# akhilsathuluri/sim_a_splat

Hardware: AMD Instinct MI355X
Metric: rendered frames/sec at 1M Gaussians 1920x1080 (higher is better)
Workload: dtype f32

## Files before the change

### sim_a_splat_amd/csrc/sas_api.cpp

```cpp
#include "../../include/sim_a_splat_amd.h"
#include "sas_internal.h"

#include <cmath>
#include <cstdarg>
#include <cstdio>
#include <cstdlib>
#include <cstring>
#include <algorithm>
#include <new>
#include <string>
#include <vector>

#pragma clang fp contract(off)

namespace {

template <class T, auto Free>
struct Owned {
    T h{};
    Owned() = default;
    Owned(Owned &&o) noexcept : h(o.h) { o.h = T{}; }
    Owned &operator=(Owned &&o) noexcept { std::swap(h, o.h); return *this; }
    ~Owned() { if (h) (void)Free(h); }
    T *put() { return &h; }
    operator T() const { return h; }
};
using Stream = Owned<hipStream_t, hipStreamDestroy>;
using Event = Owned<hipEvent_t, hipEventDestroy>;
template <class T> using Pinned = Owned<T *, hipHostFree>;

struct DevBuf {
    void *p = nullptr;
    size_t bytes = 0;
    DevBuf() = default;
    DevBuf(DevBuf &&o) noexcept : p(o.p), bytes(o.bytes) { o.p = nullptr; o.bytes = 0; }
    DevBuf &operator=(DevBuf &&o) noexcept { std::swap(p, o.p); std::swap(bytes, o.bytes); return *this; }
    ~DevBuf() { (void)release(); }
    int release(sas_ctx *c = nullptr);
};

struct ViewOut {
    float *rgb = nullptr, *alpha = nullptr, *depth = nullptr;
    uint8_t *rgb8 = nullptr;
    float *points = nullptr;
    uint8_t *mask = nullptr;
    uint8_t *rgb8_host = nullptr;
    float *features = nullptr;
    uint8_t *labels = nullptr;
    const uint8_t *lift_labels = nullptr;
    int64_t *lift_votes = nullptr, *lift_seen = nullptr;
    int lift_n = 0;
};

struct RenderArgs {
    float viewmat[16], K[9], bg[3];
// ... 213 lines not shown

uint32_t hilbert3(uint32_t x, uint32_t y, uint32_t z, int bits)
{
    uint32_t X[3] = {x, y, z};
    const uint32_t M = 1u << (bits - 1);
    for (uint32_t Q = M; Q > 1; Q >>= 1) {
        const uint32_t P = Q - 1;
        for (int i = 0; i < 3; ++i) {
            if (X[i] & Q) X[0] ^= P;
            else { const uint32_t t = (X[0] ^ X[i]) & P; X[0] ^= t; X[i] ^= t; }
        }
    }
    X[1] ^= X[0];
    X[2] ^= X[1];
    uint32_t t = 0;
    for (uint32_t Q = M; Q > 1; Q >>= 1)
        if (X[2] & Q) t ^= Q - 1;
    for (int i = 0; i < 3; ++i) X[i] ^= t;
    uint32_t code = 0;
    for (int b = bits - 1; b >= 0; --b)
        for (int i = 0; i < 3; ++i) code = (code << 1) | ((X[i] >> b) & 1u);
    return code;
}

void storage_order(int64_t n, const float *means, const uint8_t *gid, std::vector<int> &perm)
{
    perm.resize((size_t)n);
    float lo[3] = {INFINITY, INFINITY, INFINITY}, hi[3] = {-INFINITY, -INFINITY, -INFINITY};
    for (int64_t i = 0; i < n; ++i)
        for (int k = 0; k < 3; ++k) {
            const float v = means[3 * i + k];
            if (std::isfinite(v)) { lo[k] = std::min(lo[k], v); hi[k] = std::max(hi[k], v); }
        }
    float inv[3];
    for (int k = 0; k < 3; ++k) inv[k] = (hi[k] > lo[k]) ? 1023.0f / (hi[k] - lo[k]) : 0.0f;
    std::vector<uint64_t> key((size_t)n);
    for (int64_t i = 0; i < n; ++i) {
        uint32_t q[3];
        for (int k = 0; k < 3; ++k) {
            const float v = means[3 * i + k];
            float u = std::isfinite(v) ? (v - lo[k]) * inv[k] : 0.0f;
            u = std::min(std::max(u, 0.0f), 1023.0f);
            q[k] = (uint32_t)u;
        }
        const uint64_t g = gid ? gid[i] : 0;
        key[(size_t)i] = (g << 32) | hilbert3(q[0], q[1], q[2], 10);
    }
    for (int64_t i = 0; i < n; ++i) perm[(size_t)i] = (int)i;
    std::sort(perm.begin(), perm.end(), [&](int a, int b) { return key[a] != key[b] ? key[a] < key[b] : a < b; });
}

void make_cam(const float *V, const float *K, int W, int H, int tile_px, SasCam &c)
{
    for (int i = 0; i < 3; ++i) {
        for (int j = 0; j < 3; ++j) c.R[3 * i + j] = V[4 * i + j];
        c.t[i] = V[4 * i + 3];
    }
    for (int i = 0; i < 3; ++i) {
        float d = fmaf(c.R[6 + i], c.t[2], fmaf(c.R[3 + i], c.t[1], c.R[0 + i] * c.t[0]));
        c.campos[i] = -d;
    }
    c.fx = K[0]; c.fy = K[4]; c.cx = K[2]; c.cy = K[5];
    c.W = W; c.H = H;
    c.tile_px = tile_px;
    c.tw = (W + tile_px - 1) / tile_px;
    c.th = (H + tile_px - 1) / tile_px;
    c.Wf = (float)W; c.Hf = (float)H;
    const float tan_fovx = (0.5f * c.Wf) / c.fx;
    const float tan_fovy = (0.5f * c.Hf) / c.fy;
    c.lim_x_pos = fmaf(0.3f, tan_fovx, (c.Wf - c.cx) / c.fx);
    c.lim_x_neg = fmaf(0.3f, tan_fovx, c.cx / c.fx);
    c.lim_y_pos = fmaf(0.3f, tan_fovy, (c.Hf - c.cy) / c.fy);
    c.lim_y_neg = fmaf(0.3f, tan_fovy, c.cy / c.fy);
}

static size_t f_wg_stride(const sas_ctx *c) { return (((size_t)((c->scene.n + 255) / 256) + 3) & ~(size_t)3) + 4; }

int tiles_of(const Slot &sl) { return sl.cam.tw * sl.cam.th; }

long long frame_cap(const Slot &sl) { return sl.direct ? (long long)tiles_of(sl) * sl.scr.seg : sl.scr.cap; }

size_t key_slots(const Slot &sl) { return (size_t)std::max(frame_cap(sl), sl.scr.cap); }

long long grown(long long need, long long slack) { return need + need / 4 + slack; }

SasFrame frame_of(sas_ctx *c, Slot &sl, bool keep_info = false)
{
    Scratch &q = sl.scr;
    const int tiles = tiles_of(sl);
    SasFrame f{};
    f.rec = (float4 *)q.rec.p;
    f.col = (float4 *)q.col.p;
    f.info = (uint4 *)q.info.p;
    f.tickets = (unsigned *)q.counters.p;
    f.stats = (unsigned *)q.counters.p + SAS_TICKET_INTS;
    f.class_cursor = (int *)q.counters.p + SAS_TICKET_INTS + 8;
    f.stats_host = sl.stats_host;
    f.tile_count = (int *)q.counters.p + SAS_TICKET_INTS + 32;
    f.tile_big = f.tile_count + sas_count_stride(tiles);
    f.wg_base = (int *)q.wgbase.p;
    const size_t ts = sas_tile_stride(tiles);
    f.tile_offset = (int *)q.tilebuf.p;
    f.tile_cursor = (int *)q.tilebuf.p + ts;
    f.tile_order = (int *)q.tilebuf.p + 2 * ts;
    f.sort_class = (int *)q.tilebuf.p + 3 * ts;
    f.keys = (unsigned long long *)q.keys.p;
// ... 560 lines not shown
    if (n > 0 && (!means || !opacities || !colors)) return fail(c, SAS_ERR_INVALID, "means/opacities/colors required");
    const bool quat_mode = quats && scales;
    if (n > 0 && !quat_mode && !cov6) return fail(c, SAS_ERR_INVALID, "need quats+scales or cov6");
    if (n_groups < 0 || n_groups > 256) return fail(c, SAS_ERR_INVALID, "n_groups %d out of [0,256]", n_groups);
    if (group_id && n_groups <= 0) return fail(c, SAS_ERR_INVALID, "group_id given but n_groups == 0");
    HIP_TRY(c, hipSetDevice(c->device));
    if (const int rc = complete_all(c)) return rc;
    forget(c, HAVE_SCENE);

    const int deg = sh_degree < 0 ? -1 : sh_degree;
    const int coeff_floats = deg < 0 ? 3 : 3 * (deg + 1) * (deg + 1);
    const int planes = (coeff_floats + 3) / 4;
    const int64_t n_pad = (n + 63) & ~63ll;
    int rc;
    const size_t np = (size_t)(n_pad > 0 ? n_pad : 64);
    if ((rc = ensure(c, c->g0, sizeof(float4) * np))) return rc;
    if ((rc = ensure(c, c->g1, sizeof(float4) * np))) return rc;
    if ((rc = ensure(c, c->g2, sizeof(float4) * np))) return rc;
    if ((rc = ensure(c, c->col, sizeof(float4) * np * planes))) return rc;
    if ((rc = ensure(c, c->gid8, np))) return rc;

    c->perm_host.clear();
    if ((rc = ensure(c, c->perm, sizeof(int) * np))) return rc;
    if (n > 0) {
        std::vector<float> h_means((size_t)3 * n);
        std::vector<uint8_t> h_gid;
        HIP_TRY(c, hipMemcpy(h_means.data(), means, sizeof(float) * 3 * n, hipMemcpyDefault));
        if (group_id) {
            h_gid.resize((size_t)n);
            HIP_TRY(c, hipMemcpy(h_gid.data(), group_id, (size_t)n, hipMemcpyDefault));
            for (int64_t i = 0; i < n; ++i)
                if (h_gid[(size_t)i] >= n_groups) return fail(c, SAS_ERR_INVALID, "group_id[%lld]=%d >= n_groups=%d", (long long)i, (int)h_gid[(size_t)i], n_groups);
        }
        storage_order(n, h_means.data(), group_id ? h_gid.data() : nullptr, c->perm_host);
        HIP_TRY(c, hipMemcpy(c->perm.p, c->perm_host.data(), sizeof(int) * n, hipMemcpyHostToDevice));

        DevBuf s_means, s_q, s_s, s_cov, s_op, s_col, s_gid;
        auto stage = [&](DevBuf &b, const void *src, size_t bytes) -> int {
            if (const int rc = ensure(c, b, bytes)) return rc;
            HIP_TRY(c, hipMemcpy(b.p, src, bytes, hipMemcpyDefault));
            return SAS_OK;
        };
        rc = stage(s_means, means, sizeof(float) * 3 * n);
        if (!rc && quat_mode) rc = stage(s_q, quats, sizeof(float) * 4 * n);
        if (!rc && quat_mode) rc = stage(s_s, scales, sizeof(float) * 3 * n);
        if (!rc && !quat_mode) rc = stage(s_cov, cov6, sizeof(float) * 6 * n);
        if (!rc) rc = stage(s_op, opacities, sizeof(float) * n);
        if (!rc) rc = stage(s_col, colors, sizeof(float) * (size_t)coeff_floats * n);
        if (!rc && group_id) rc = stage(s_gid, group_id, (size_t)n);
        if (!rc) {
            sas_launch_relayout(nullptr, n, n_pad, (const int *)c->perm.p, (const float *)s_means.p,
                                (const float *)s_q.p, (const float *)s_s.p, (const float *)s_cov.p,
                                (const float *)s_op.p, (const float *)s_col.p, coeff_floats, planes,
                                (const uint8_t *)s_gid.p, (float4 *)c->g0.p, (float4 *)c->g1.p, (float4 *)c->g2.p,
                                (float4 *)c->col.p, (uint8_t *)c->gid8.p);
            hipError_t e = hipDeviceSynchronize();
            if (e != hipSuccess) rc = fail(c, SAS_ERR_HIP, "relayout: %s", hipGetErrorString(e));
        }
        if (rc) return rc;
    }

    c->scene = SasScene{};
    c->scene.g0 = (const float4 *)c->g0.p;
    c->scene.g1 = (const float4 *)c->g1.p;
    c->scene.g2 = (const float4 *)c->g2.p;
    c->scene.col = (const float4 *)c->col.p;
    c->scene.gid8 = (const uint8_t *)c->gid8.p;
    c->scene.perm = (const int *)c->perm.p;
    c->scene.n = n;
    c->scene.n_pad = n_pad;
    c->scene.sh_degree = deg;
    c->scene.cov_mode = quat_mode ? 0 : 1;
    c->scene.n_groups = group_id ? n_groups : 0;
    c->group_host.clear();
    c->links = LinkConsts{};
    if (group_id) {
        c->group_host.assign((size_t)12 * n_groups, 0.0f);
        for (int g = 0; g < n_groups; ++g) c->group_host[12 * g + 0] = c->group_host[12 * g + 5] = c->group_host[12 * g + 10] = 1.0f;
    }
    for (Slot &sl : c->slots) sl.scr.cap = 0;
    c->has_frame = false;
    c->scene_version++;
    c->have |= HAVE_SCENE;
    return SAS_OK;
}

int sas_set_group_poses(sas_ctx *c, int n_groups, const float *Rt)
{
    if (!c || !Rt) return SAS_ERR_INVALID;
    if (!has(c, HAVE_SCENE)) return fail(c, SAS_ERR_NO_SCENE, "no scene uploaded");
    if (n_groups != c->scene.n_groups) return fail(c, SAS_ERR_INVALID, "scene has %d groups, got %d", c->scene.n_groups, n_groups);
    c->group_host.assign(Rt, Rt + (size_t)12 * n_groups);
    return SAS_OK;
}

namespace {

void quat_to_matrix(const double *qin, double *R)
{
    const double n = std::sqrt(qin[0] * qin[0] + qin[1] * qin[1] + qin[2] * qin[2] + qin[3] * qin[3]);
    const double q[4] = {qin[0] / n, qin[1] / n, qin[2] / n, qin[3] / n};
    double qq[4][4];
    for (int a = 0; a < 4; ++a)
        for (int b = 0; b < 4; ++b) qq[a][b] = q[a] * q[b];
    R[0] = 1 - 2 * (qq[2][2] + qq[3][3]); R[1] = 2 * (qq[1][2] - qq[0][3]); R[2] = 2 * (qq[1][3] + qq[0][2]);
    R[3] = 2 * (qq[1][2] + qq[0][3]); R[4] = 1 - 2 * (qq[1][1] + qq[3][3]); R[5] = 2 * (qq[2][3] - qq[0][1]);
    R[6] = 2 * (qq[1][3] - qq[0][2]); R[7] = 2 * (qq[2][3] + qq[0][1]); R[8] = 1 - 2 * (qq[1][1] + qq[2][2]);
}

void matrix_to_quat(const double *R, double *q)
{
    const double tr = R[0] + R[4] + R[8];
    if (tr > 0) {
        const double s = std::sqrt(tr + 1.0) * 2;
        q[0] = 0.25 * s; q[1] = (R[7] - R[5]) / s; q[2] = (R[2] - R[6]) / s; q[3] = (R[3] - R[1]) / s;
    } else {
        int i = 0;
        if (R[4] > R[0]) i = 1;
        if (R[8] > R[4 * i]) i = 2;
        const int j = (i + 1) % 3, k = (i + 2) % 3;
        const double s = std::sqrt(1.0 + R[4 * i] - R[4 * j] - R[4 * k]) * 2;
        q[0] = (R[3 * k + j] - R[3 * j + k]) / s;
        q[1 + i] = 0.25 * s;
        q[1 + j] = (R[3 * j + i] + R[3 * i + j]) / s;
        q[1 + k] = (R[3 * k + i] + R[3 * i + k]) / s;
// ... 1126 lines not shown
```

### sim_a_splat_amd/csrc/sas_device.h

```cpp
#pragma once
#include "sas_internal.h"

#pragma clang fp contract(off)

#define DEV __device__ __forceinline__

constexpr float kNear = 0.01f, kFar = 1e10f, kEps2d = 0.3f;
constexpr float kAlphaThr = 1.0f / 255.0f, kMaxAlpha = 0.999f, kTStop = 1e-4f;

DEV float fma_(float a, float b, float c) { return __builtin_fmaf(a, b, c); }
DEV float finite_colour(float v) { return fminf(fmaxf(v, -3.402823466e38f), 3.402823466e38f); }
DEV unsigned mbcnt64(unsigned long long m) { return __builtin_amdgcn_mbcnt_hi((unsigned)(m >> 32), __builtin_amdgcn_mbcnt_lo((unsigned)m, 0u)); }

#ifdef SAS_DEBUG_BOUNDS
static __device__ unsigned long long g_sas_bounds[4];
DEV bool sas_in_bounds(long long i, long long n, int code)
{
    if (i >= 0 && i < n) return true;
    if (atomicAdd(&g_sas_bounds[0], 1ull) == 0ull) {
        g_sas_bounds[1] = (unsigned long long)code;
        g_sas_bounds[2] = (unsigned long long)i;
        g_sas_bounds[3] = (unsigned long long)n;
    }
    return false;
// ... 65 lines not shown
    unsigned u = __float_as_uint(x);
    int e = (int)(u >> 23) - 127;
    float m = __uint_as_float((u & 0x007fffffu) | 0x3f800000u);
    if (m > 1.41421356237f) { m = m * 0.5f; e += 1; }
    float s = (m - 1.0f) / (m + 1.0f);
    float s2 = s * s;
    float p = 0.1111111111f;
    p = fma_(p, s2, 0.1428571429f);
    p = fma_(p, s2, 0.2f);
    p = fma_(p, s2, 0.3333333333f);
    p = fma_(p, s2, 1.0f);
    float lnm = (2.0f * s) * p;
    return fma_((float)e, 0.6931471805599453f, lnm);
}

DEV float affine3(float r0, float r1, float r2, float t, float v0, float v1, float v2)
{
    return fma_(r0, v0, fma_(r1, v1, fma_(r2, v2, t)));
}
DEV float dot3(float a0, float a1, float a2, float b0, float b1, float b2)
{
    return fma_(a2, b2, fma_(a1, b1, a0 * b0));
}
DEV void pose_point(const float *G, float *p)
{
    const float x = affine3(G[0], G[1], G[2], G[3], p[0], p[1], p[2]);
    const float y = affine3(G[4], G[5], G[6], G[7], p[0], p[1], p[2]);
    const float z = affine3(G[8], G[9], G[10], G[11], p[0], p[1], p[2]);
    p[0] = x; p[1] = y; p[2] = z;
}
DEV void to_camera(const SasCam &c, const float *p, float *q)
{
    q[0] = affine3(c.R[0], c.R[1], c.R[2], c.t[0], p[0], p[1], p[2]);
    q[1] = affine3(c.R[3], c.R[4], c.R[5], c.t[1], p[0], p[1], p[2]);
    q[2] = affine3(c.R[6], c.R[7], c.R[8], c.t[2], p[0], p[1], p[2]);
}

DEV void rot_sym3(const float *R, const float *s, float *out)
{
    const float S[3][3] = {{s[0], s[1], s[2]}, {s[1], s[3], s[4]}, {s[2], s[4], s[5]}};
    float T[3][3];
#pragma unroll
    for (int i = 0; i < 3; ++i)
#pragma unroll
        for (int j = 0; j < 3; ++j)
            T[i][j] = dot3(R[3 * i + 0], R[3 * i + 1], R[3 * i + 2], S[0][j], S[1][j], S[2][j]);
    out[0] = dot3(T[0][0], T[0][1], T[0][2], R[0], R[1], R[2]);
    out[1] = dot3(T[0][0], T[0][1], T[0][2], R[3], R[4], R[5]);
    out[2] = dot3(T[0][0], T[0][1], T[0][2], R[6], R[7], R[8]);
    out[3] = dot3(T[1][0], T[1][1], T[1][2], R[3], R[4], R[5]);
    out[4] = dot3(T[1][0], T[1][1], T[1][2], R[6], R[7], R[8]);
    out[5] = dot3(T[2][0], T[2][1], T[2][2], R[6], R[7], R[8]);
}
```

### sim_a_splat_amd/csrc/sas_internal.h

```cpp
#pragma once
#include <hip/hip_runtime.h>
#include <stdint.h>

#define SAS_TILE 16
#define SAS_RS 2
#define SAS_CS 1
#define SAS_MAX_GROUP 4

struct SasCam {
    float R[9], t[3];
    float campos[3];
    float fx, fy, cx, cy;
    float lim_x_pos, lim_x_neg, lim_y_pos, lim_y_neg;
    float Wf, Hf;
    int W, H, tw, th;
    int tile_px;
};

struct SasScene {
    const float4 *g0, *g1, *g2, *col;
    const uint8_t *gid8;
    const int *perm;
    int64_t n;
    int64_t n_pad;
    int sh_degree;
    int cov_mode;
    int n_groups;
};

struct SasFrame {
    float4 *rec;
    float4 *col;
    uint4 *info;
    int *tile_count;
    int *tile_big;
    int *wg_base;
    int *class_cursor;
    int *tile_offset;
    int *tile_cursor;
    int *tile_order;
    int *sort_class;
    unsigned long long *keys;
    int *sorted_ids;
    long long cap;
    int seg;
    int cull;
    int group_fill;
    int keep_info;
    unsigned *stats;
    unsigned *tickets;
    unsigned *stats_host;
    int *wg_vis;
    int *wg_isect16;
    unsigned *tile_max;
    const float *group_Rt;
    const float *group_host;
    int n_wg;
    int n_tiles;
};

struct SasOutputs {
    float *rgb, *alpha, *depth;
    uint8_t *rgb8;
    uint8_t *rgb8_host;
    float bg[3];
    float *points;
    uint8_t *mask;
    float max_depth;
    int use_max_depth;
    long long n_pixels;
};
// ... 28 lines not shown
};
void sas_launch_pose_upload(hipStream_t st, const SasPoseUpload &u);

struct SasHostCopy {
    int nv;
    const uint8_t *src[SAS_MAX_GROUP];
    uint8_t *dst[SAS_MAX_GROUP];
    size_t bytes;
};
void sas_launch_host_copy(hipStream_t st, const SasHostCopy &h);

#define SAS_FEAT_K 8
#define SAS_MAX_FEATURES 256
struct SasFeatures {
    const float *store;
    float *out;
    long long n_pad;
    int C, chunks;
    float bg[SAS_MAX_FEATURES];
};
static inline int sas_feature_chunks(int C) { return (C + SAS_FEAT_K - 1) / SAS_FEAT_K; }
void sas_launch_feature_store(hipStream_t st, int64_t n, int64_t n_pad, const int *perm, const uint8_t *gid8, const float *src,
                              int C, float *store);
struct SasMeshFeatures {
    const unsigned long long *win;
    const float *store;
    long long nt;
};
void sas_launch_blend_features(hipStream_t st, const SasScene &s, int tiles, const SasParams &P, const SasFrame &f,
                               const SasFeatures &F, bool fast_exp, const SasMeshFeatures *MF);
struct SasLabels {
    const float *store;
    long long n_pad;
    int C, chunks;
    uint8_t *out;
    float min_alpha;
    int surface;
};
void sas_launch_blend_labels(hipStream_t st, const SasScene &s, int tiles, const SasParams &P, const SasFrame &f, const SasLabels &B,
                             bool fast_exp, const SasMeshFeatures *MF);
struct SasLift {
    const uint8_t *labels;
    unsigned long long *votes;
    unsigned long long *seen;
    long long n;
    int n_labels;
};
void sas_launch_lift_labels(hipStream_t st, const SasScene &s, int tiles, const SasParams &P, const SasFrame &f, const SasLift &B,
                            bool fast_exp);
void sas_launch_mesh_feature_store(hipStream_t st, int64_t nt, const int4 *tri, const float *src, int C, float *store);

void sas_launch_relayout(hipStream_t st, int64_t n, int64_t n_pad, const int *perm, const float *means, const float *quats,
                         const float *scales, const float *cov6, const float *opac, const float *colors,
                         int coeff_floats, int planes, const uint8_t *gid, float4 *g0, float4 *g1, float4 *g2,
                         float4 *col, uint8_t *gid8);
void sas_launch_project(hipStream_t st, const SasScene &s, const SasParams &P, const SasFrame &f);
void sas_launch_project2(hipStream_t st, const SasScene &s, const SasParams &P0, const SasFrame &f0, const SasParams &P1,
                         const SasFrame &f1);
void sas_launch_project_multi(hipStream_t st, const SasScene &s, const SasMulti &mf);
void sas_launch_scatter_multi(hipStream_t st, const SasScene &s, int tw, const SasMulti &mf);
void sas_launch_tiles_lazy_multi(hipStream_t st, const SasScene &s, int tiles, const SasMulti &mf, bool fast_exp, bool want_max,
                                 bool quad, hipEvent_t ev_start, hipEvent_t ev_stop);
void sas_launch_scatter(hipStream_t st, const SasScene &s, int tw, const SasFrame &f);
struct SasSortStreams {
    hipStream_t side[2];
    hipEvent_t fork, join[2];
};
void sas_launch_sort(hipStream_t st, const SasScene &s, int tiles, const SasFrame &f, const SasSortStreams &ss);
void sas_launch_blend(hipStream_t st, const SasScene &s, int tiles, const SasParams &P, const SasFrame &f,
                      bool fast_exp, bool want_max);
bool sas_tiles_lazy_quad_ok(bool fast_exp);
void sas_launch_tiles_lazy(hipStream_t st, const SasScene &s, int tiles, const SasParams &P, const SasFrame &f,
                           bool fast_exp, bool want_max, bool quad, hipEvent_t ev_start, hipEvent_t ev_stop);
void sas_launch_depth_tail(hipStream_t st, int tiles, const SasParams &P, const SasFrame &f, bool fill, bool points);
#define SAS_TICKET_INTS (65 * 32)
#define SAS_WIN_BINS 2048
static inline size_t sas_count_stride(int tiles) { return (((size_t)tiles + 1 + 1023) & ~(size_t)1023) + 1024; }
static inline size_t sas_counter_ints(int tiles) { return SAS_TICKET_INTS + 32 + 2 * sas_count_stride(tiles); }
static inline size_t sas_tile_stride(int tiles) { return ((size_t)tiles + 1 + 3) & ~(size_t)3; }

struct SasMeshScene {
    const float4 *vert;
    const int4 *tri;
    const float4 *color;
    int nv, nt;
    int n_groups;
    float ka, kd;
    const float4 *vnormal;
    const float4 *vcolor;
};
struct SasMeshFrame {
    float4 *rec;
    int4 *rect;
    int *tile_count;
    int *tile_offset;
    int *tile_cursor;
    int *list;
    long long cap;
    int n_rec;
    unsigned *status_host;
};
struct SasMeshExtra {
    unsigned long long *win;
    int surface;
};
#define SAS_MESH_PLANE_STRIDE 3
void sas_launch_mesh_bin(hipStream_t st, const SasMeshScene &m, const SasParams &P, const SasFrame &f, const SasMeshFrame &mf,
// ... 102 lines not shown
```

### sim_a_splat_amd/csrc/sas_kernels.hip

```cpp
#include "sas_device.h"

#include <cstdlib>
#include <cstring>
#include <type_traits>

#pragma clang fp contract(off)

namespace {

__global__ __launch_bounds__(256) void k_relayout(int64_t n, int64_t n_pad, const int *perm, const float *means,
                                                  const float *quats, const float *scales, const float *cov6,
                                                  const float *opac, const float *colors, int coeff_floats, int planes,
                                                  const uint8_t *gid, float4 *g0, float4 *g1, float4 *g2, float4 *col, uint8_t *gid8)
{
    const int64_t j = (int64_t)blockIdx.x * 256 + threadIdx.x;
    if (j >= n) return;
    const int64_t i = perm[j];
    float gbits = __uint_as_float(gid ? (unsigned)gid[i] : 0u);
    gid8[j] = gid ? gid[i] : (uint8_t)0;
    g0[j] = make_float4(means[3 * i], means[3 * i + 1], means[3 * i + 2], opac[i]);
    if (quats) {
        g1[j] = make_float4(quats[4 * i], quats[4 * i + 1], quats[4 * i + 2], quats[4 * i + 3]);
        g2[j] = make_float4(scales[3 * i], scales[3 * i + 1], scales[3 * i + 2], gbits);
    } else {
        const float *c = cov6 + 6 * i;
        g1[j] = make_float4(c[0], c[1], c[2], c[3]);
        g2[j] = make_float4(c[4], c[5], 0.0f, gbits);
    }
    const float *src = colors + (int64_t)coeff_floats * i;
    for (int p = 0; p < planes; ++p) {
        float v[4];
#pragma unroll
        for (int k = 0; k < 4; ++k) v[k] = (4 * p + k < coeff_floats) ? src[4 * p + k] : 0.0f;
        col[(int64_t)p * n_pad + j] = make_float4(v[0], v[1], v[2], v[3]);
    }
}

template <int DEG>
DEV void sh_to_color(const float *sh, float dx, float dy, float dz, float *rgb)
{
    float inorm = 1.0f / sqrtf(fma_(dz, dz, fma_(dy, dy, dx * dx)));
    float x = dx * inorm, y = dy * inorm, z = dz * inorm;
    float r[3];
#pragma unroll
    for (int c = 0; c < 3; ++c) r[c] = 0.2820947917738781f * sh[0 * 3 + c];
    if constexpr (DEG >= 1) {
#pragma unroll
        for (int c = 0; c < 3; ++c) {
            float t = fma_(-x, sh[3 * 3 + c], fma_(z, sh[2 * 3 + c], (-y) * sh[1 * 3 + c]));
            r[c] = fma_(0.48860251190292f, t, r[c]);
        }
    }
    float z2 = z * z;
    float fC1 = fma_(x, x, -(y * y));
    float fS1 = 2.0f * x * y;
    if constexpr (DEG >= 2) {
        float fTmp0B = -1.092548430592079f * z;
        float pSH6 = fma_(0.9461746957575601f, z2, -0.3153915652525201f);
        float pSH7 = fTmp0B * x;
        float pSH5 = fTmp0B * y;
        float pSH8 = 0.5462742152960395f * fC1;
        float pSH4 = 0.5462742152960395f * fS1;
#pragma unroll
        for (int c = 0; c < 3; ++c) {
            r[c] = fma_(pSH4, sh[4 * 3 + c], r[c]);
            r[c] = fma_(pSH5, sh[5 * 3 + c], r[c]);
            r[c] = fma_(pSH6, sh[6 * 3 + c], r[c]);
            r[c] = fma_(pSH7, sh[7 * 3 + c], r[c]);
            r[c] = fma_(pSH8, sh[8 * 3 + c], r[c]);
        }
    }
    if constexpr (DEG >= 3) {
        float fTmp0C = fma_(-2.285228997322329f, z2, 0.4570457994644658f);
        float fTmp1B = 1.445305721320277f * z;
        float fC2 = fma_(x, fC1, -(y * fS1));
        float fS2 = fma_(x, fS1, y * fC1);
        float pSH12 = z * fma_(1.865881662950577f, z2, -1.119528997770346f);
        float pSH13 = fTmp0C * x;
        float pSH11 = fTmp0C * y;
        float pSH14 = fTmp1B * fC1;
        float pSH10 = fTmp1B * fS1;
// ... 131 lines not shown
};

DEV Window window_of(int X0, int Y0, int X1, int Y1)
{
    Window w;
    w.X0 = X0; w.Y0 = Y0;
    w.ww = X1 - X0;
    w.area = (X1 > X0 && Y1 > Y0) ? w.ww * (Y1 - Y0) : 0;
    w.fits = w.area > 0 && w.area <= kHistBins;
    return w;
}

DEV Window wg_window(bool part, int x0, int x1, int y0, int y1, int *s_win)
{
    int mnx = part ? x0 : 0x7fffffff, mny = part ? y0 : 0x7fffffff;
    int mxx = part ? x1 : 0, mxy = part ? y1 : 0;
    mnx = wave_min_i32(mnx); mny = wave_min_i32(mny);
    mxx = wave_max_i32(mxx); mxy = wave_max_i32(mxy);
    if (threadIdx.x == 0) { s_win[0] = 0x7fffffff; s_win[1] = 0x7fffffff; s_win[2] = 0; s_win[3] = 0; }
    __syncthreads();
    if ((threadIdx.x & 63) == 0) {
        atomicMin(&s_win[0], mnx); atomicMin(&s_win[1], mny);
        atomicMax(&s_win[2], mxx); atomicMax(&s_win[3], mxy);
    }
    __syncthreads();
    return window_of(s_win[0], s_win[1], s_win[2], s_win[3]);
}

DEV Window wg_window_zeroed(bool part, int x0, int x1, int y0, int y1, int *s_win16, int *s_hist)
{
    int mnx = part ? x0 : 0x7fffffff, mny = part ? y0 : 0x7fffffff;
    int mxx = part ? x1 : 0, mxy = part ? y1 : 0;
    mnx = wave_min_i32(mnx); mny = wave_min_i32(mny);
    mxx = wave_max_i32(mxx); mxy = wave_max_i32(mxy);
    if ((threadIdx.x & 63) == 0) *reinterpret_cast<int4 *>(s_win16 + 4 * (threadIdx.x >> 6)) = make_int4(mnx, mny, mxx, mxy);
    static_assert(kHistBins == 2048, "eight bins per thread");
    reinterpret_cast<int4 *>(s_hist)[threadIdx.x] = make_int4(0, 0, 0, 0);
    reinterpret_cast<int4 *>(s_hist)[256 + threadIdx.x] = make_int4(0, 0, 0, 0);
    __syncthreads();
    const int4 a = reinterpret_cast<const int4 *>(s_win16)[0], b = reinterpret_cast<const int4 *>(s_win16)[1],
               c = reinterpret_cast<const int4 *>(s_win16)[2], d = reinterpret_cast<const int4 *>(s_win16)[3];
    return window_of(min(min(a.x, b.x), min(c.x, d.x)), min(min(a.y, b.y), min(c.y, d.y)),
                     max(max(a.z, b.z), max(c.z, d.z)), max(max(a.w, b.w), max(c.w, d.w)));
}

DEV bool mean_survives(float cz, float op) { return !(cz < kNear || cz > kFar) && !(op < kAlphaThr); }

struct ViewGeom {
    bool vis;
    int x0, x1, y0, y1;
    float mx, my, ca, cb, ccn, thr, z, rx, ry;
};

DEV void project_view(const SasCam &c, const float *cov, float op, float x, float y, float z, ViewGeom &g)
{
    float cc3[6];
    rot_sym3(c.R, cov, cc3);

    const float rz = 1.0f / z;
    const float rz2 = rz * rz;
    const float tx = z * fminf(c.lim_x_pos, fmaxf(-c.lim_x_neg, x * rz));
    const float ty = z * fminf(c.lim_y_pos, fmaxf(-c.lim_y_neg, y * rz));
    const float ja = c.fx * rz, jb = -((c.fx * tx) * rz2);
    const float jc = c.fy * rz, jd = -((c.fy * ty) * rz2);
    const float t00 = fma_(jb, cc3[2], ja * cc3[0]);
    const float t01 = fma_(jb, cc3[4], ja * cc3[1]);
    const float t02 = fma_(jb, cc3[5], ja * cc3[2]);
    const float t11 = fma_(jd, cc3[4], jc * cc3[3]);
    const float t12 = fma_(jd, cc3[5], jc * cc3[4]);
    float c00 = fma_(t02, jb, t00 * ja);
    const float c01 = fma_(t02, jd, t01 * jc);
    float c11 = fma_(t12, jd, t11 * jc);
    const float mx = fma_(c.fx, x * rz, c.cx);
    const float my = fma_(c.fy, y * rz, c.cy);
    c00 += kEps2d;
    c11 += kEps2d;
    const float det = fma_(c00, c11, -(c01 * c01));
    if (!(det > 0.0f)) return;
    const float inv_det = 1.0f / det;
    const float ca = c11 * inv_det, cb = -c01 * inv_det, ccn = c00 * inv_det;
    const float lnq = c_logf(op / kAlphaThr);
    const float extent = fminf(3.33f, sqrtf(2.0f * lnq));
    const float b = 0.5f * (c00 + c11);
    const float tmp = sqrtf(fmaxf(0.01f, fma_(b, b, -det)));
    const float v1 = b + tmp;
    const float r1 = extent * sqrtf(v1);
    const float rx = ceilf(fminf(extent * sqrtf(c00), r1));
    const float ry = ceilf(fminf(extent * sqrtf(c11), r1));
    bool keep = !(rx <= 0.0f && ry <= 0.0f);
    keep = keep && !(mx + rx <= 0.0f || mx - rx >= c.Wf || my + ry <= 0.0f || my - ry >= c.Hf);
    keep = keep && rx > 0.0f && ry > 0.0f;
    if (!keep) return;
    g.vis = true;
    const float ts = (float)c.tile_px;
    const float trx = rx / ts, try_ = ry / ts;
    const float ttx = mx / ts, tty = my / ts;
    const float twf = (float)c.tw, thf = (float)c.th;
    g.x0 = (int)fminf(fmaxf(floorf(ttx - trx), 0.0f), twf);
    g.x1 = (int)fminf(fmaxf(ceilf(ttx + trx), 0.0f), twf);
    g.y0 = (int)fminf(fmaxf(floorf(tty - try_), 0.0f), thf);
    g.y1 = (int)fminf(fmaxf(ceilf(tty + try_), 0.0f), thf);
    if (c.tile_px == 8 && !(op <= 1.0f)) {
        g.x0 &= ~1; g.y0 &= ~1;
        g.x1 = min((g.x1 + 1) & ~1, c.tw); g.y1 = min((g.y1 + 1) & ~1, c.th);
    }
    g.mx = mx; g.my = my; g.ca = ca; g.cb = cb; g.ccn = ccn; g.z = z; g.rx = rx; g.ry = ry;
    const float t = lnq + 1e-3f;
    g.thr = t < 85.9f ? t : __builtin_inff();
}

struct CullGeom {
    float mx, my, ha, b, hc, nba, nbc, lim;
};
DEV CullGeom cull_geom(const ViewGeom &g)
{
    return CullGeom{g.mx, g.my, 0.5f * g.ca, g.cb, 0.5f * g.ccn, -g.cb / g.ca, -g.cb / g.ccn, g.thr + 0.05f};
}
struct CullRow {
    float ly, hy, dyc, c2, t, bdyc;
};
DEV CullRow cull_row(const CullGeom &q, int ty, float px)
{
    CullRow r;
    r.ly = ((float)ty * px + 0.5f) - q.my;
    r.hy = r.ly + (px - 1.0f);
    r.dyc = __builtin_amdgcn_fmed3f(0.0f, r.ly, r.hy);
    r.c2 = q.hc * r.dyc * r.dyc;
    r.t = q.nba * r.dyc;
    r.bdyc = q.b * r.dyc;
    return r;
}
DEV bool tile_reached(const CullGeom &q, const CullRow &r, int tx, float px)
{
    const float lx = ((float)tx * px + 0.5f) - q.mx, hx = lx + (px - 1.0f);
    const float dxc = __builtin_amdgcn_fmed3f(0.0f, lx, hx);
    const float dys = __builtin_amdgcn_fmed3f(q.nbc * dxc, r.ly, r.hy), dxs = __builtin_amdgcn_fmed3f(r.t, lx, hx);
    const float t1 = q.ha * dxc, t3 = q.hc * dys;
    const float s1 = fma_(t1, dxc, t3 * dys);
    const float q1 = fma_(q.b * dxc, dys, s1);
    const float m1 = fma_(-2e-5f, s1, q1);
    const float s2 = fma_(q.ha * dxs, dxs, r.c2);
    const float q2 = fma_(r.bdyc, dxs, s2);
    const float m2 = fma_(-2e-5f, s2, q2);
    return !(m1 > q.lim && m2 > q.lim);
}
DEV bool tile_reached(const CullGeom &q, int tx, int ty, float px) { return tile_reached(q, cull_row(q, ty, px), tx, px); }
template <typename F>
DEV void for_each_reached_tile(bool active, bool cull, const CullGeom &q, float px, int x0, int x1, int y0, int y1, int tw,
                               unsigned v0, unsigned v1, F emit)
// ... 415 lines not shown
        }
    }
    __syncthreads();
    if (tid < 16) {
        int sum = 0;
        for (int k = 0; k < 32; ++k) sum += s_bins[32 * tid + k];
        s_w[tid] = sum;
    }
    __syncthreads();
    if (tid == 0) tail_publish(f, s_w, carry, (long long)carry > f.cap , nvis_all, n16_all, maxlen_all);
}

template <int NV>
DEV float4 scene_load(const float4 *p)
{
    if constexpr (NV >= 2) return nt_load(p);
    else return *p;
}

template <typename RowFn>
DEV bool group_pose(unsigned gid, const float *poses, bool poses_inline, RowFn inline_row, float *G)
{
    if (poses_inline) {
        unsigned long long todo = __ballot(true);
        while (todo) {
            const unsigned g = (unsigned)__builtin_amdgcn_readlane((int)gid, __ffsll((long long)todo) - 1);
            const bool mine = gid == g;
#pragma unroll
            for (int k = 0; k < 12; ++k) {
                const float r = inline_row(g, k);
                if (mine) G[k] = r;
            }
            todo &= ~__ballot(mine);
        }
        return true;
    }
    if (poses) {
        const float *Gp = poses + 12 * gid;
#pragma unroll
        for (int k = 0; k < 12; ++k) G[k] = Gp[k];
        return true;
    }
    return false;
}

struct ProjArgs {
    SasCam cam[2];
    SasFrame f[2];
    int mix_k;
    int pose_inline;
    float pose_rows[12 * kProjInlineRows];
};

DEV void world_covariance(bool cov_mode, const float4 &a1, const float4 &a2, bool hasG, const float *G, float *cov)
{
    if (!cov_mode) {
        float qw = a1.x, qx = a1.y, qy = a1.z, qz = a1.w;
        float n2 = fma_(qz, qz, fma_(qy, qy, fma_(qx, qx, qw * qw)));
        float inv = 1.0f / sqrtf(n2);
        qw *= inv; qx *= inv; qy *= inv; qz *= inv;
        float x2 = qx * qx, y2 = qy * qy, z2 = qz * qz;
        float xy = qx * qy, xz = qx * qz, yz = qy * qz;
        float wx = qw * qx, wy = qw * qy, wz = qw * qz;
        float R[9];
        R[0] = fma_(-2.0f, y2 + z2, 1.0f); R[1] = 2.0f * (xy - wz);           R[2] = 2.0f * (xz + wy);
        R[3] = 2.0f * (xy + wz);           R[4] = fma_(-2.0f, x2 + z2, 1.0f); R[5] = 2.0f * (yz - wx);
        R[6] = 2.0f * (xz - wy);           R[7] = 2.0f * (yz + wx);           R[8] = fma_(-2.0f, x2 + y2, 1.0f);
        if (hasG) {
            float R2[9];
#pragma unroll
            for (int r = 0; r < 3; ++r)
#pragma unroll
                for (int k = 0; k < 3; ++k)
                    R2[3 * r + k] = dot3(G[4 * r + 0], G[4 * r + 1], G[4 * r + 2], R[0 + k], R[3 + k], R[6 + k]);
#pragma unroll
            for (int k = 0; k < 9; ++k) R[k] = R2[k];
        }
        const float sc[3] = {a2.x, a2.y, a2.z};
        float M[9];
#pragma unroll
        for (int r = 0; r < 3; ++r)
#pragma unroll
            for (int k = 0; k < 3; ++k) M[3 * r + k] = R[3 * r + k] * sc[k];
        cov[0] = dot3(M[0], M[1], M[2], M[0], M[1], M[2]);
        cov[1] = dot3(M[0], M[1], M[2], M[3], M[4], M[5]);
        cov[2] = dot3(M[0], M[1], M[2], M[6], M[7], M[8]);
        cov[3] = dot3(M[3], M[4], M[5], M[3], M[4], M[5]);
        cov[4] = dot3(M[3], M[4], M[5], M[6], M[7], M[8]);
        cov[5] = dot3(M[6], M[7], M[8], M[6], M[7], M[8]);
    } else {
        cov[0] = a1.x; cov[1] = a1.y; cov[2] = a1.z; cov[3] = a1.w; cov[4] = a2.x; cov[5] = a2.y;
        if (hasG) {
            const float Rg[9] = {G[0], G[1], G[2], G[4], G[5], G[6], G[8], G[9], G[10]};
            float c2[6];
            rot_sym3(Rg, cov, c2);
#pragma unroll
            for (int k = 0; k < 6; ++k) cov[k] = c2[k];
        }
    }
}

DEV bool last_workgroup_of_view(const SasFrame &f, unsigned wg, int *s_last, ProjLap &pl_)
{
    asm volatile("s_waitcnt vmcnt(0)" ::: "memory");
    __syncthreads();
    PL_LAP(7);
    if (threadIdx.x == 0) {
        unsigned *tk = f.tickets;
        const unsigned n_wg = (unsigned)f.n_wg;
        const unsigned sub = wg & 63u, n_sub = (n_wg - sub + 63u) >> 6, subs = min(n_wg, 64u);
        int last = 0;
        if (atomicAdd(&tk[32u * sub], 1u) == n_sub - 1u) {
            tk[32u * sub] = 0u;
            last = atomicAdd(&tk[32u * 64u], 1u) == subs - 1u;
            if (last) tk[32u * 64u] = 0u;
        }
        *s_last = last;
    }
    __syncthreads();
    PL_LAP(8);
    return *s_last != 0;
}

DEV void view_tail(const SasFrame &f, int *lds, ProjLap &pl_)
{
    __builtin_amdgcn_fence(__ATOMIC_ACQUIRE, "agent");
    if (f.seg > 0) scan_tail_single(&f, lds, pl_);
    else scan_tail_two_pass(&f, lds);
}

template <typename RowFn>
DEV void geom_role(const SasScene &s, const SasCam &c, const SasFrame &f, unsigned wg, const float *poses, bool poses_inline,
                   RowFn inline_row, const ProjLds &L)
{
    const int64_t i = (int64_t)wg * 256 + threadIdx.x;
    ProjLap pl_{wg, 0ull};
#ifdef SAS_TUNE_PTIME
    pl_.t = wall_clock64();
    if (threadIdx.x == 0 && wg < (unsigned)kDbgPMax) g_dbg_plap[16 * wg + 14] = pl_.t;
#endif
    ViewGeom g;
    g.vis = false; g.x0 = g.x1 = g.y0 = g.y1 = 0; g.z = 0.0f;
    if (i < s.n) {
        const float4 a0 = s.g0[i];
        const float4 a1 = s.g1[i];
        const float4 a2 = s.g2[i];
        float m[3] = {a0.x, a0.y, a0.z};
        const float op = a0.w;
        float G[12] = {1.f, 0.f, 0.f, 0.f, 0.f, 1.f, 0.f, 0.f, 0.f, 0.f, 1.f, 0.f};
        const bool hasG = group_pose(__float_as_uint(a2.w) & 255u, poses, poses_inline, inline_row, G);
        if (hasG) pose_point(G, m);
        float q[3];
        to_camera(c, m, q);
        if (mean_survives(q[2], op)) {
            float cov[6];
            world_covariance(s.cov_mode != 0, a1, a2, hasG, G, cov);
            project_view(c, cov, op, q[0], q[1], q[2], g);
        }
        if (g.vis) {
            f.rec[SAS_RS * i + 0] = make_float4(g.mx, g.my, g.ca, g.cb);
            f.rec[SAS_RS * i + 1] = make_float4(g.ccn, op, g.thr, g.z);
            const int irx = (int)fminf(g.rx, 2147483520.0f), iry = (int)fminf(g.ry, 2147483520.0f);
            if (f.keep_info) f.info[i] = make_uint4((unsigned)g.x0 | ((unsigned)g.x1 << 16), (unsigned)g.y0 | ((unsigned)g.y1 << 16), (unsigned)irx, (unsigned)iry);
        } else if (f.keep_info) {
            f.info[i] = make_uint4(0u, 0u, 0u, 0u);
        }
    }
    PL_LAP(0);
    count_tiles(f, c.tw, c.tile_px, g, (unsigned)i, wg, L, pl_);
    const bool last = last_workgroup_of_view(f, wg, L.last, pl_);
#ifdef SAS_TUNE_PTIME
    if (threadIdx.x == 0 && wg < (unsigned)kDbgPMax) g_dbg_plap[16 * wg + 15] = wall_clock64();
#endif
    if (!last) return;
    view_tail(f, L.hist, pl_);
    PL_LAP(9);
#ifdef SAS_TUNE_PTIME
    if (threadIdx.x == 0 && wg < (unsigned)kDbgPMax) g_dbg_plap[16 * wg + 15] = wall_clock64();
#endif
}

template <int DEG, int NV, typename RowFn>
DEV void color_role(const SasScene &s, const ProjArgs &vs, unsigned wg, const float *poses, bool poses_inline, RowFn inline_row)
{
    const int64_t i = (int64_t)wg * 256 + threadIdx.x;
#ifdef SAS_TUNE_PTIME
    if (threadIdx.x == 0 && wg < (unsigned)kDbgPMax) g_dbg_pcol[2 * wg] = wall_clock64();
#endif
    if (i >= s.n) return;
    const float4 a0 = s.g0[i];
    float m[3] = {a0.x, a0.y, a0.z};
    const float op = a0.w;
    if (s.n_groups > 0) {
        float G[12] = {1.f, 0.f, 0.f, 0.f, 0.f, 1.f, 0.f, 0.f, 0.f, 0.f, 1.f, 0.f};
        if (group_pose((unsigned)s.gid8[i], poses, poses_inline, inline_row, G)) pose_point(G, m);
    }
    bool ok[NV], any_ok = false;
#pragma unroll
    for (int v = 0; v < NV; ++v) {
        float q[3];
        to_camera(vs.cam[v], m, q);
        ok[v] = mean_survives(q[2], op);
        any_ok = any_ok || ok[v];
    }
    if (!any_ok) return;
    if constexpr (DEG == 3) {
        float a[24];
#pragma unroll
        for (int p = 0; p < 6; ++p) {
            const float4 q = scene_load<NV>(s.col + (int64_t)p * s.n_pad + i);
// ... 176 lines not shown
        order_body(f, (int)blockIdx.x);
        return;
    }
    const unsigned wg = blockIdx.x - (unsigned)n_order;
    __shared__ int s_win[4];
    __shared__ int s_hist[kHistBins];
    __shared__ int s_base[kHistBins];
    const int64_t i = (int64_t)wg * 256 + threadIdx.x;
    uint4 inf = make_uint4(0u, 0u, 0u, 0u);
    if (i < s.n) inf = f.info[i];
    const int x0 = inf.x & 0xffff, x1 = inf.x >> 16, y0 = inf.y & 0xffff, y1 = inf.y >> 16;
    const bool vis = x1 > x0 && y1 > y0;
    const unsigned zbits = vis ? __float_as_uint(f.rec[SAS_RS * i + 1].w) : 0u;
    const unsigned long long key = ((unsigned long long)zbits << 32) | (unsigned long long)(unsigned)i;
    const int rect_area = vis ? (x1 - x0) * (y1 - y0) : 0;
    const bool in_win = rect_area > 0 && rect_area <= kWinRect;
    const Window w = wg_window(in_win, x0, x1, y0, y1, s_win);
    if (w.fits) {
        const int *wb = f.wg_base + (size_t)wg * SAS_WIN_BINS;
        for_each_window_bin(w, tw, [&](unsigned b, int tile) {
            s_base[b] = SAS_IN(tile, f.n_tiles, 112) ? f.tile_offset[tile] + wb[b] : 0;
            s_hist[b] = 0;
        });
        __syncthreads();
        if (in_win)
#pragma unroll 1
            for (int ty = y0; ty < y1; ++ty)
#pragma unroll 1
                for (int tx = x0; tx < x1; ++tx) {
                    const int b = (ty - w.Y0) * w.ww + (tx - w.X0);
                    if (!SAS_IN(b, kHistBins, 113)) continue;
                    const long long pos = (long long)s_base[b] + atomicAdd(&s_hist[b], 1);
                    if (pos < f.cap && SAS_IN(pos, (long long)f.tile_offset[ty * tw + tx + 1], 114)) f.keys[pos] = key;
                }
    }
    const unsigned klo = (unsigned)key, khi = (unsigned)(key >> 32);
    for_each_tile(vis && !(w.fits && in_win), x0, x1, y0, y1, tw, klo, khi, [&](int tile, unsigned lo, unsigned hi) {
        if (!SAS_IN(tile, f.n_tiles, 115)) return;
        const int pos = atomicAdd(&f.tile_cursor[tile], 1);
        if ((long long)pos < f.cap && SAS_IN(pos, f.tile_offset[tile + 1], 116)) f.keys[pos] = ((unsigned long long)hi << 32) | lo;
    });
}

#define SAS_SCATTER_ATTRS __launch_bounds__(256) __attribute__((amdgpu_num_vgpr(32)))
__global__ SAS_SCATTER_ATTRS void k_scatter(SasScene s, int tw, SasFrame f) { scatter_body(s, tw, f); }
__global__ SAS_SCATTER_ATTRS void k_scatter_multi(SasScene s, int tw, SasMulti mf) { scatter_body(s, tw, mf.f[blockIdx.y]); }

}

SAS_BOUNDS_ACCESSOR(sas_debug_bounds_kernels)

void sas_launch_relayout(hipStream_t st, int64_t n, int64_t n_pad, const int *perm, const float *means, const float *quats,
                         const float *scales, const float *cov6, const float *opac, const float *colors,
                         int coeff_floats, int planes, const uint8_t *gid, float4 *g0, float4 *g1, float4 *g2,
                         float4 *col, uint8_t *gid8)
{
    if (n <= 0) return;
    const unsigned grid = (unsigned)((n + 255) / 256);
    hipLaunchKernelGGL(k_relayout, dim3(grid), dim3(256), 0, st, n, n_pad, perm, means, quats, scales, cov6, opac, colors,
                       coeff_floats, planes, gid, g0, g1, g2, col, gid8);
}

static unsigned sas_spread_blocks(unsigned n_wg) { return 16u * ((n_wg + 15u) / 16u); }
static int project_mix(int nv, unsigned n_wg)
{
    static const int env = [] { const char *e = getenv("SAS_PROJ_MIX"); return e ? atoi(e) : 0; }();
    const unsigned n_geo = (unsigned)nv * sas_spread_blocks(n_wg), total = n_geo + n_wg;
    const int kmin = (int)((8u * n_geo + total - 1u) / total);
    const int k = env > 0 ? env : (nv == 1 ? 5 : 7);
    return k < kmin ? kmin : (k > 8 ? 8 : k);
}

extern "C" int sas_debug_projection_block(unsigned b, unsigned n_wg, int nv, unsigned *out)
{
    if (!out || n_wg == 0 || nv < 1 || nv > 2) return -1;
    const unsigned n_geo = (unsigned)nv * sas_spread_blocks(n_wg), grid = n_geo + n_wg;
    const unsigned mix = (unsigned)project_mix(nv, n_wg);
    out[0] = grid;
    out[1] = mix;
    if (b >= grid) return -2;
    const Role r = block_role(b, (unsigned)nv * kSpreadRows * spread_cols(n_wg), mix);
    out[2] = r.geom ? 1u : 0u;
    out[3] = r.geom ? spread_chunk(nv == 1 ? r.idx : r.idx >> 1, n_wg) : r.idx;
    out[4] = (r.geom && nv == 2) ? (r.idx & 1u) : 0u;
    return 0;
}

template <typename Fn>
static void with_degree(int sh_degree, Fn fn)
{
    switch (sh_degree) {
        case 0: fn(std::integral_constant<int, 0>{}); break;
        case 1: fn(std::integral_constant<int, 1>{}); break;
        case 2: fn(std::integral_constant<int, 2>{}); break;
        case 3: fn(std::integral_constant<int, 3>{}); break;
        default: fn(std::integral_constant<int, -1>{}); break;
    }
}

template <int NV>
static void launch_project(hipStream_t st, const SasScene &s, const ProjArgs &vs)
{
    const unsigned n_wg = (unsigned)vs.f[0].n_wg;
    const unsigned grid = (unsigned)NV * sas_spread_blocks(n_wg) + n_wg;
    with_degree(s.sh_degree, [&](auto deg) { hipLaunchKernelGGL((k_project<decltype(deg)::value, NV>), dim3(grid), dim3(256), 0, st, s, vs); });
}

static void inline_poses(ProjArgs &vs, const SasScene &s)
{
    vs.pose_inline = sas_poses_inline(s.n_groups, 1, false) && vs.f[0].group_host ? 1 : 0;
    if (vs.pose_inline) memcpy(vs.pose_rows, vs.f[0].group_host, sizeof(float) * 12 * (size_t)s.n_groups);
}

// ... 76 lines not shown
```

Before: 7211.

## Precompute world covariance and opacity terms at upload for static scenes

For scenes with no group ids, the relayout kernel now computes the world-space covariance and the opacity log/extent terms once at upload and stores them in the g1/g2 slots. The per-frame projection then reads them directly instead of normalising quaternions, building rotations and calling log/sqrt for every Gaussian. The per-tile division is also replaced by a multiply with a constant reciprocal, and an assert restricts tile size to 8 or 16. The trade-off is a new scene mode that drops the group-id bits from g2 and has to be kept consistent with every path that reads it.

```diff
diff --git a/sim_a_splat_amd/csrc/sas_api.cpp b/sim_a_splat_amd/csrc/sas_api.cpp
--- a/sim_a_splat_amd/csrc/sas_api.cpp
+++ b/sim_a_splat_amd/csrc/sas_api.cpp
@@ -1,6 +1,7 @@
 #include "../../include/sim_a_splat_amd.h"
 #include "sas_internal.h"
 
+#include <cassert>
 #include <cmath>
 #include <cstdarg>
 #include <cstdio>
@@ -320,6 +321,7 @@
 
 void make_cam(const float *V, const float *K, int W, int H, int tile_px, SasCam &c)
 {
+    assert(tile_px == 8 || tile_px == 16);
     for (int i = 0; i < 3; ++i) {
         for (int j = 0; j < 3; ++j) c.R[3 * i + j] = V[4 * i + j];
         c.t[i] = V[4 * i + 3];
@@ -986,7 +988,7 @@
             sas_launch_relayout(nullptr, n, n_pad, (const int *)c->perm.p, (const float *)s_means.p,
                                 (const float *)s_q.p, (const float *)s_s.p, (const float *)s_cov.p,
                                 (const float *)s_op.p, (const float *)s_col.p, coeff_floats, planes,
-                                (const uint8_t *)s_gid.p, (float4 *)c->g0.p, (float4 *)c->g1.p, (float4 *)c->g2.p,
+                                (const uint8_t *)s_gid.p,  !group_id, (float4 *)c->g0.p, (float4 *)c->g1.p, (float4 *)c->g2.p,
                                 (float4 *)c->col.p, (uint8_t *)c->gid8.p);
             hipError_t e = hipDeviceSynchronize();
             if (e != hipSuccess) rc = fail(c, SAS_ERR_HIP, "relayout: %s", hipGetErrorString(e));
@@ -1004,7 +1006,7 @@
     c->scene.n = n;
     c->scene.n_pad = n_pad;
     c->scene.sh_degree = deg;
-    c->scene.cov_mode = quat_mode ? 0 : 1;
+    c->scene.cov_mode = !group_id ? kSceneStatic : quat_mode ? kSceneQuatScale : kSceneCov;
     c->scene.n_groups = group_id ? n_groups : 0;
     c->group_host.clear();
     c->links = LinkConsts{};
diff --git a/sim_a_splat_amd/csrc/sas_device.h b/sim_a_splat_amd/csrc/sas_device.h
--- a/sim_a_splat_amd/csrc/sas_device.h
+++ b/sim_a_splat_amd/csrc/sas_device.h
@@ -141,3 +141,57 @@
     out[4] = dot3(T[1][0], T[1][1], T[1][2], R[6], R[7], R[8]);
     out[5] = dot3(T[2][0], T[2][1], T[2][2], R[6], R[7], R[8]);
 }
+
+DEV void world_covariance(bool cov_mode, const float4 &a1, const float4 &a2, bool hasG, const float *G, float *cov)
+{
+    if (!cov_mode) {
+        float qw = a1.x, qx = a1.y, qy = a1.z, qz = a1.w;
+        float n2 = fma_(qz, qz, fma_(qy, qy, fma_(qx, qx, qw * qw)));
+        float inv = 1.0f / sqrtf(n2);
+        qw *= inv; qx *= inv; qy *= inv; qz *= inv;
+        float x2 = qx * qx, y2 = qy * qy, z2 = qz * qz;
+        float xy = qx * qy, xz = qx * qz, yz = qy * qz;
+        float wx = qw * qx, wy = qw * qy, wz = qw * qz;
+        float R[9];
+        R[0] = fma_(-2.0f, y2 + z2, 1.0f); R[1] = 2.0f * (xy - wz);           R[2] = 2.0f * (xz + wy);
+        R[3] = 2.0f * (xy + wz);           R[4] = fma_(-2.0f, x2 + z2, 1.0f); R[5] = 2.0f * (yz - wx);
+        R[6] = 2.0f * (xz - wy);           R[7] = 2.0f * (yz + wx);           R[8] = fma_(-2.0f, x2 + y2, 1.0f);
+        if (hasG) {
+            float R2[9];
+#pragma unroll
+            for (int r = 0; r < 3; ++r)
+#pragma unroll
+                for (int k = 0; k < 3; ++k)
+                    R2[3 * r + k] = dot3(G[4 * r + 0], G[4 * r + 1], G[4 * r + 2], R[0 + k], R[3 + k], R[6 + k]);
+#pragma unroll
+            for (int k = 0; k < 9; ++k) R[k] = R2[k];
+        }
+        const float sc[3] = {a2.x, a2.y, a2.z};
+        float M[9];
+#pragma unroll
+        for (int r = 0; r < 3; ++r)
+#pragma unroll
+            for (int k = 0; k < 3; ++k) M[3 * r + k] = R[3 * r + k] * sc[k];
+        cov[0] = dot3(M[0], M[1], M[2], M[0], M[1], M[2]);
+        cov[1] = dot3(M[0], M[1], M[2], M[3], M[4], M[5]);
+        cov[2] = dot3(M[0], M[1], M[2], M[6], M[7], M[8]);
+        cov[3] = dot3(M[3], M[4], M[5], M[3], M[4], M[5]);
+        cov[4] = dot3(M[3], M[4], M[5], M[6], M[7], M[8]);
+        cov[5] = dot3(M[6], M[7], M[8], M[6], M[7], M[8]);
+    } else {
+        cov[0] = a1.x; cov[1] = a1.y; cov[2] = a1.z; cov[3] = a1.w; cov[4] = a2.x; cov[5] = a2.y;
+        if (hasG) {
+            const float Rg[9] = {G[0], G[1], G[2], G[4], G[5], G[6], G[8], G[9], G[10]};
+            float c2[6];
+            rot_sym3(Rg, cov, c2);
+#pragma unroll
+            for (int k = 0; k < 6; ++k) cov[k] = c2[k];
+        }
+    }
+}
+
+DEV void opacity_terms(float op, float &lnq, float &extent)
+{
+    lnq = c_logf(op / kAlphaThr);
+    extent = fminf(3.33f, sqrtf(2.0f * lnq));
+}
diff --git a/sim_a_splat_amd/csrc/sas_internal.h b/sim_a_splat_amd/csrc/sas_internal.h
--- a/sim_a_splat_amd/csrc/sas_internal.h
+++ b/sim_a_splat_amd/csrc/sas_internal.h
@@ -17,6 +17,7 @@
     int tile_px;
 };
 
+enum { kSceneQuatScale = 0, kSceneCov = 1, kSceneStatic = 2 };
 struct SasScene {
     const float4 *g0, *g1, *g2, *col;
     const uint8_t *gid8;
@@ -151,7 +152,7 @@
 
 void sas_launch_relayout(hipStream_t st, int64_t n, int64_t n_pad, const int *perm, const float *means, const float *quats,
                          const float *scales, const float *cov6, const float *opac, const float *colors,
-                         int coeff_floats, int planes, const uint8_t *gid, float4 *g0, float4 *g1, float4 *g2,
+                         int coeff_floats, int planes, const uint8_t *gid, bool static_terms, float4 *g0, float4 *g1, float4 *g2,
                          float4 *col, uint8_t *gid8);
 void sas_launch_project(hipStream_t st, const SasScene &s, const SasParams &P, const SasFrame &f);
 void sas_launch_project2(hipStream_t st, const SasScene &s, const SasParams &P0, const SasFrame &f0, const SasParams &P1,
diff --git a/sim_a_splat_amd/csrc/sas_kernels.hip b/sim_a_splat_amd/csrc/sas_kernels.hip
--- a/sim_a_splat_amd/csrc/sas_kernels.hip
+++ b/sim_a_splat_amd/csrc/sas_kernels.hip
@@ -11,7 +11,8 @@
 __global__ __launch_bounds__(256) void k_relayout(int64_t n, int64_t n_pad, const int *perm, const float *means,
                                                   const float *quats, const float *scales, const float *cov6,
                                                   const float *opac, const float *colors, int coeff_floats, int planes,
-                                                  const uint8_t *gid, float4 *g0, float4 *g1, float4 *g2, float4 *col, uint8_t *gid8)
+                                                  const uint8_t *gid, int static_terms, float4 *g0, float4 *g1, float4 *g2, float4 *col,
+                                                  uint8_t *gid8)
 {
     const int64_t j = (int64_t)blockIdx.x * 256 + threadIdx.x;
     if (j >= n) return;
@@ -19,14 +20,24 @@
     float gbits = __uint_as_float(gid ? (unsigned)gid[i] : 0u);
     gid8[j] = gid ? gid[i] : (uint8_t)0;
     g0[j] = make_float4(means[3 * i], means[3 * i + 1], means[3 * i + 2], opac[i]);
+    float4 a1, a2;
     if (quats) {
-        g1[j] = make_float4(quats[4 * i], quats[4 * i + 1], quats[4 * i + 2], quats[4 * i + 3]);
-        g2[j] = make_float4(scales[3 * i], scales[3 * i + 1], scales[3 * i + 2], gbits);
+        a1 = make_float4(quats[4 * i], quats[4 * i + 1], quats[4 * i + 2], quats[4 * i + 3]);
+        a2 = make_float4(scales[3 * i], scales[3 * i + 1], scales[3 * i + 2], gbits);
     } else {
         const float *c = cov6 + 6 * i;
-        g1[j] = make_float4(c[0], c[1], c[2], c[3]);
-        g2[j] = make_float4(c[4], c[5], 0.0f, gbits);
-    }
+        a1 = make_float4(c[0], c[1], c[2], c[3]);
+        a2 = make_float4(c[4], c[5], 0.0f, gbits);
+    }
+    if (static_terms) {
+        float cov[6], lnq, extent;
+        world_covariance(quats == nullptr, a1, a2, false, nullptr, cov);
+        opacity_terms(opac[i], lnq, extent);
+        a1 = make_float4(cov[0], cov[1], cov[2], cov[3]);
+        a2 = make_float4(cov[4], cov[5], lnq, extent);
+    }
+    g1[j] = a1;
+    g2[j] = a2;
     const float *src = colors + (int64_t)coeff_floats * i;
     for (int p = 0; p < planes; ++p) {
         float v[4];
@@ -264,7 +275,8 @@
     float mx, my, ca, cb, ccn, thr, z, rx, ry;
 };
 
-DEV void project_view(const SasCam &c, const float *cov, float op, float x, float y, float z, ViewGeom &g)
+DEV void project_view(const SasCam &c, const float *cov, float op, bool static_terms, float lnq_s, float extent_s, float x, float y, float z,
+                      ViewGeom &g)
 {
     float cc3[6];
     rot_sym3(c.R, cov, cc3);
@@ -291,8 +303,8 @@
     if (!(det > 0.0f)) return;
     const float inv_det = 1.0f / det;
     const float ca = c11 * inv_det, cb = -c01 * inv_det, ccn = c00 * inv_det;
-    const float lnq = c_logf(op / kAlphaThr);
-    const float extent = fminf(3.33f, sqrtf(2.0f * lnq));
+    float lnq = lnq_s, extent = extent_s;
+    if (!static_terms) opacity_terms(op, lnq, extent);
     const float b = 0.5f * (c00 + c11);
     const float tmp = sqrtf(fmaxf(0.01f, fma_(b, b, -det)));
     const float v1 = b + tmp;
@@ -304,9 +316,9 @@
     keep = keep && rx > 0.0f && ry > 0.0f;
     if (!keep) return;
     g.vis = true;
-    const float ts = (float)c.tile_px;
-    const float trx = rx / ts, try_ = ry / ts;
-    const float ttx = mx / ts, tty = my / ts;
+    const float its = c.tile_px == 8 ? 0.125f : 0.0625f;
+    const float trx = rx * its, try_ = ry * its;
+    const float ttx = mx * its, tty = my * its;
     const float twf = (float)c.tw, thf = (float)c.th;
     g.x0 = (int)fminf(fmaxf(floorf(ttx - trx), 0.0f), twf);
     g.x1 = (int)fminf(fmaxf(ceilf(ttx + trx), 0.0f), twf);
@@ -828,54 +840,6 @@
     float pose_rows[12 * kProjInlineRows];
 };
 
-DEV void world_covariance(bool cov_mode, const float4 &a1, const float4 &a2, bool hasG, const float *G, float *cov)
-{
-    if (!cov_mode) {
-        float qw = a1.x, qx = a1.y, qy = a1.z, qz = a1.w;
-        float n2 = fma_(qz, qz, fma_(qy, qy, fma_(qx, qx, qw * qw)));
-        float inv = 1.0f / sqrtf(n2);
-        qw *= inv; qx *= inv; qy *= inv; qz *= inv;
-        float x2 = qx * qx, y2 = qy * qy, z2 = qz * qz;
-        float xy = qx * qy, xz = qx * qz, yz = qy * qz;
-        float wx = qw * qx, wy = qw * qy, wz = qw * qz;
-        float R[9];
-        R[0] = fma_(-2.0f, y2 + z2, 1.0f); R[1] = 2.0f * (xy - wz);           R[2] = 2.0f * (xz + wy);
-        R[3] = 2.0f * (xy + wz);           R[4] = fma_(-2.0f, x2 + z2, 1.0f); R[5] = 2.0f * (yz - wx);
-        R[6] = 2.0f * (xz - wy);           R[7] = 2.0f * (yz + wx);           R[8] = fma_(-2.0f, x2 + y2, 1.0f);
-        if (hasG) {
-            float R2[9];
-#pragma unroll
-            for (int r = 0; r < 3; ++r)
-#pragma unroll
-                for (int k = 0; k < 3; ++k)
-                    R2[3 * r + k] = dot3(G[4 * r + 0], G[4 * r + 1], G[4 * r + 2], R[0 + k], R[3 + k], R[6 + k]);
-#pragma unroll
-            for (int k = 0; k < 9; ++k) R[k] = R2[k];
-        }
-        const float sc[3] = {a2.x, a2.y, a2.z};
-        float M[9];
-#pragma unroll
-        for (int r = 0; r < 3; ++r)
-#pragma unroll
-            for (int k = 0; k < 3; ++k) M[3 * r + k] = R[3 * r + k] * sc[k];
-        cov[0] = dot3(M[0], M[1], M[2], M[0], M[1], M[2]);
-        cov[1] = dot3(M[0], M[1], M[2], M[3], M[4], M[5]);
-        cov[2] = dot3(M[0], M[1], M[2], M[6], M[7], M[8]);
-        cov[3] = dot3(M[3], M[4], M[5], M[3], M[4], M[5]);
-        cov[4] = dot3(M[3], M[4], M[5], M[6], M[7], M[8]);
-        cov[5] = dot3(M[6], M[7], M[8], M[6], M[7], M[8]);
-    } else {
-        cov[0] = a1.x; cov[1] = a1.y; cov[2] = a1.z; cov[3] = a1.w; cov[4] = a2.x; cov[5] = a2.y;
-        if (hasG) {
-            const float Rg[9] = {G[0], G[1], G[2], G[4], G[5], G[6], G[8], G[9], G[10]};
-            float c2[6];
-            rot_sym3(Rg, cov, c2);
-#pragma unroll
-            for (int k = 0; k < 6; ++k) cov[k] = c2[k];
-        }
-    }
-}
-
 DEV bool last_workgroup_of_view(const SasFrame &f, unsigned wg, int *s_last, ProjLap &pl_)
 {
     asm volatile("s_waitcnt vmcnt(0)" ::: "memory");
@@ -924,14 +888,19 @@
         float m[3] = {a0.x, a0.y, a0.z};
         const float op = a0.w;
         float G[12] = {1.f, 0.f, 0.f, 0.f, 0.f, 1.f, 0.f, 0.f, 0.f, 0.f, 1.f, 0.f};
-        const bool hasG = group_pose(__float_as_uint(a2.w) & 255u, poses, poses_inline, inline_row, G);
+        const bool stat = s.cov_mode == kSceneStatic;
+        const bool hasG = group_pose(stat ? 0u : __float_as_uint(a2.w) & 255u, poses, poses_inline, inline_row, G);
         if (hasG) pose_point(G, m);
         float q[3];
         to_camera(c, m, q);
         if (mean_survives(q[2], op)) {
             float cov[6];
-            world_covariance(s.cov_mode != 0, a1, a2, hasG, G, cov);
-            project_view(c, cov, op, q[0], q[1], q[2], g);
+            if (stat) {
+                cov[0] = a1.x; cov[1] = a1.y; cov[2] = a1.z; cov[3] = a1.w; cov[4] = a2.x; cov[5] = a2.y;
+            } else {
+                world_covariance(s.cov_mode == kSceneCov, a1, a2, hasG, G, cov);
+            }
+            project_view(c, cov, op, stat, a2.z, a2.w, q[0], q[1], q[2], g);
         }
         if (g.vis) {
             f.rec[SAS_RS * i + 0] = make_float4(g.mx, g.my, g.ca, g.cb);
@@ -1214,13 +1183,13 @@
 
 void sas_launch_relayout(hipStream_t st, int64_t n, int64_t n_pad, const int *perm, const float *means, const float *quats,
                          const float *scales, const float *cov6, const float *opac, const float *colors,
-                         int coeff_floats, int planes, const uint8_t *gid, float4 *g0, float4 *g1, float4 *g2,
+                         int coeff_floats, int planes, const uint8_t *gid, bool static_terms, float4 *g0, float4 *g1, float4 *g2,
                          float4 *col, uint8_t *gid8)
 {
     if (n <= 0) return;
     const unsigned grid = (unsigned)((n + 255) / 256);
     hipLaunchKernelGGL(k_relayout, dim3(grid), dim3(256), 0, st, n, n_pad, perm, means, quats, scales, cov6, opac, colors,
-                       coeff_floats, planes, gid, g0, g1, g2, col, gid8);
+                       coeff_floats, planes, gid, static_terms ? 1 : 0, g0, g1, g2, col, gid8);
 }
 
 static unsigned sas_spread_blocks(unsigned n_wg) { return 16u * ((n_wg + 15u) / 16u); }
```

New measurement: 7337 (median of 6 runs). Within noise of the previous version (+1.8%).
